# leggedrobotics/wild_visual_navigation

Hardware: NVIDIA H100
Metric: frames/sec end-to-end (DINO feat + seg + MLP train-step) at 448x448 (higher is better)
Workload: dtype bf16 operands / fp32 accumulate (ViT, STEGO head, per-pixel MLP); fp32 (k-means, train step)

## Files before the change

include/wvn_b200.h:

```cpp
#ifndef WVN_B200_H_
#define WVN_B200_H_

#include <stddef.h>
#include <stdint.h>

#ifdef __cplusplus
extern "C" {
#endif

typedef enum {
  WVN_STATUS_OK = 0,
  WVN_STATUS_INVALID = -1,
  WVN_STATUS_CUDA = -2,
  WVN_STATUS_NO_DEVICE = -3,
  WVN_STATUS_STATE = -4
} wvn_status;

const char* wvn_last_error(void);
int wvn_check_device(void);
int wvn_version(void);
long long wvn_launch_count(void);
void wvn_profile_enable(int category_mask);
int wvn_profile_collect(float* host_ms, long long* host_launches);

int wvn_gemm_bf16(const void* a_bf16, long long lda, const void* w_bf16, const float* bias, void* out, long long ldo,
                  int m, int n, int k, int out_kind, int act, int block_n, void* stream);

typedef struct {
  int m, n, k;
  int epi, act;
  int block_n;
  const void* a;
  long long lda;
  const void* w;
  const float* bias;
  void* out;
  long long ldo;
  const float* pos;
  int tokens_in, npad;
  int dim, heads;
  void* q_out;
  void* k_out;
  void* vt_out;
  int feat, trav_col;
  const void* x;
  long long ldx;
  float* trav;
  float* conf;
  float* loss_reco;
  const float* cg_mean;
  const float* cg_std;
  float cg_std_factor;
  int reverse_m;
  int registers;
  const void* residual;
  long long ldr;
} wvn_gemm_ex_args;
int wvn_gemm_bf16_ex(const wvn_gemm_ex_args* args, void* stream);

int wvn_attention_bf16(const void* q, const void* k, const void* vt, void* out, int batch, int heads, int npad,
                       int n_valid, float scale, void* stream);

int wvn_layernorm(const float* x, const float* gamma, const float* beta, void* out_bf16, long long rows, int dim,
                  float eps, void* stream);

typedef struct wvn_vit wvn_vit_t;

typedef struct {
  int image_size;
  int patch_size;
  int dim;
  int depth;
  int heads;
  int mlp_dim;
  int max_batch;
  int chunk;
  float ln_eps;
  int head_out;
  int registers;
} wvn_vit_config;

int wvn_vit_create(const wvn_vit_config* cfg, wvn_vit_t** out);
void wvn_vit_destroy(wvn_vit_t* h);

int wvn_vit_set_weight(wvn_vit_t* h, const char* name, const float* data, long long numel);

int wvn_vit_forward(wvn_vit_t* h, const float* img, int batch, int in_h, int in_w, int resized_h, int resized_w,
                    float* tokens_out, void* stream);

// ... 149 lines not shown
```

wild_visual_navigation_b200/_C.py:

```python
from __future__ import annotations

import ctypes
import os
from ctypes import POINTER, Structure, byref, c_char_p, c_float, c_int, c_longlong, c_size_t, c_void_p

import torch

_HERE = os.path.dirname(os.path.abspath(__file__))
LIB_PATH = os.environ.get("WVN_B200_LIB", os.path.join(_HERE, "libwvn_b200.so"))


class WvnError(RuntimeError):
    pass


class VitConfig(Structure):
    _fields_ = [
        ("image_size", c_int), ("patch_size", c_int), ("dim", c_int), ("depth", c_int), ("heads", c_int),
        ("mlp_dim", c_int), ("max_batch", c_int), ("chunk", c_int), ("ln_eps", c_float), ("head_out", c_int),
        ("registers", c_int),
    ]


class GemmExArgs(Structure):
    _fields_ = [
        ("m", c_int), ("n", c_int), ("k", c_int), ("epi", c_int), ("act", c_int), ("block_n", c_int),
        ("a", c_void_p), ("lda", c_longlong), ("w", c_void_p), ("bias", c_void_p), ("out", c_void_p), ("ldo", c_longlong),
        ("pos", c_void_p), ("tokens_in", c_int), ("npad", c_int), ("dim", c_int), ("heads", c_int),
        ("q_out", c_void_p), ("k_out", c_void_p), ("vt_out", c_void_p),
        ("feat", c_int), ("trav_col", c_int), ("x", c_void_p), ("ldx", c_longlong), ("trav", c_void_p),
        ("conf", c_void_p), ("loss_reco", c_void_p), ("cg_mean", c_void_p), ("cg_std", c_void_p),
        ("cg_std_factor", c_float), ("reverse_m", c_int), ("registers", c_int), ("residual", c_void_p), ("ldr", c_longlong),
    ]


class ResnetConfig(Structure):
    _fields_ = [("image_size", c_int), ("depth", c_int), ("max_batch", c_int)]


class TrainConfig(Structure):
    _fields_ = [
        ("w_trav", c_float), ("w_reco", c_float), ("std_factor", c_float), ("anomaly_balanced", c_int),
        ("lr", c_float), ("beta1", c_float), ("beta2", c_float), ("eps", c_float),
    ]


class FlowBuffers(Structure):
    _fields_ = [("mask0", c_void_p), ("mask1", c_void_p), ("p1", c_void_p), ("invp1", c_void_p), ("p3", c_void_p),
                ("invp3", c_void_p)]


_lib = None

_P, _I, _L, _F, _S = c_void_p, c_int, c_longlong, c_float, c_size_t
SIGNATURES = {
    "wvn_last_error": (c_char_p, []),
    "wvn_check_device": (_I, []),
    "wvn_version": (_I, []),
    "wvn_launch_count": (_L, []),
    "wvn_profile_enable": (None, [_I]),
    "wvn_profile_collect": (_I, [_P, _P]),
    "wvn_gemm_bf16": (_I, [_P, _L, _P, _P, _P, _L, _I, _I, _I, _I, _I, _I, _P]),
    "wvn_gemm_bf16_ex": (_I, [POINTER(GemmExArgs), _P]),
    "wvn_attention_bf16": (_I, [_P, _P, _P, _P, _I, _I, _I, _I, _F, _P]),
    "wvn_layernorm": (_I, [_P, _P, _P, _P, _L, _I, _F, _P]),
# ... 108 lines not shown
```

wild_visual_navigation_b200/csrc/api.cu:

```cuda
#include <cuda_bf16.h>

#include <stdio.h>
#include <stdlib.h>

#include <map>
#include <string>
#include <vector>

#include "../../include/wvn_b200.h"
#include "attention.h"
#include "dense_kernels.h"
#include "gemm.h"
#include "host_common.h"
#include "mlp_train.h"
#include "mlp_train_fused.h"
#include "pixel_head.h"
#include "resnet_kernels.h"
#include "segment_kernels.h"
#include "flow_train.h"
#include "footprint_kernels.h"
#include "slic_kernels.h"
#include "stego_kmeans.h"
#include "train_core.h"
#include "vit_kernels.h"
// ... 54 lines not shown
};

}

struct wvn_vit {
  wvn_vit_config cfg;
  int grid = 0, P = 0, t0 = 1, n_valid = 0, npad = 0, kpe = 0, kpe_ld = 0, chunk = 0;
  std::map<std::string, Weight> w;
  std::vector<DevBuf> owned;
  DevBuf x, xn, q, k, vt, attn, hid, ape, stage;
  DevBuf tok_bf16, head_hidden;
  DevBuf qkv_f32;
  bool precise = false;
  bool forwarded = false;
  int last_batch = 0;

  int add_weight(const std::string& name, long long numel, bool bf16, int cols = 0, int ld = 0) {
    DevBuf b;
    const long long stored = cols > 0 ? numel / cols * ld : numel;
    WVN_PROPAGATE(b.alloc(static_cast<size_t>(stored) * (bf16 ? 2 : 4)));
    owned.push_back(b);
    Weight wt;
    wt.p = b.p; wt.numel = numel; wt.bf16 = bf16; wt.cols = cols; wt.ld = ld;
    w[name] = wt;
    return WVN_OK;
  }
  template <class T>
  T* wp(const std::string& name) { return reinterpret_cast<T*>(w[name].p); }
};

extern "C" {

const char* wvn_last_error(void) { return last_error(); }
int wvn_version(void) { return 104; }

int wvn_check_device(void) {
  int n = 0;
  if (cudaGetDeviceCount(&n) != cudaSuccess || n == 0) return set_error(WVN_ERR_NO_DEVICE, "no CUDA device visible");
  int dev = 0;
  cudaGetDevice(&dev);
  int major = 0;
  cudaDeviceGetAttribute(&major, cudaDevAttrComputeCapabilityMajor, dev);
  int minor = 0;
  cudaDeviceGetAttribute(&minor, cudaDevAttrComputeCapabilityMinor, dev);
  if (major != 9 || minor != 0)
    return set_error(WVN_ERR_NO_DEVICE, "device %d has compute capability %d.%d, need 9.0 (sm_90a)", dev, major, minor);
  return WVN_OK;
}

long long wvn_launch_count(void) { return launch_count(); }
void wvn_profile_enable(int category_mask) { prof_enable(category_mask); }
int wvn_profile_collect(float* host_ms, long long* host_launches) {
  WVN_REQUIRE(host_ms && host_launches, "wvn_profile_collect: null argument");
  return prof_collect(host_ms, host_launches);
}

int wvn_gemm_bf16(const void* a, long long lda, const void* w, const float* bias, void* out, long long ldo, int m, int n,
                  int k, int out_kind, int act, int block_n, void* stream) {
  GemmArgs g;
  g.M = m; g.N = n; g.K = k;
  g.epi = out_kind == 0 ? EPI_BF16 : (out_kind == 1 ? EPI_F32 : EPI_RESID_F32);
  WVN_REQUIRE(out_kind >= 0 && out_kind <= 2, "wvn_gemm_bf16: out_kind %d", out_kind);
  g.act = act; g.bias = bias; g.out = out; g.ldo = ldo;
  return gemm_bf16(g, a, lda, w, block_n, S(stream));
}

int wvn_gemm_bf16_ex(const wvn_gemm_ex_args* x, void* stream) {
  WVN_REQUIRE(x, "wvn_gemm_bf16_ex: null argument");
  GemmArgs g;
  g.M = x->m; g.N = x->n; g.K = x->k; g.epi = x->epi; g.act = x->act;
  g.bias = x->bias; g.out = x->out; g.ldo = x->ldo;
  g.pos = x->pos; g.tokens_in = x->tokens_in; g.npad = x->npad;
  g.dim = x->dim; g.heads = x->heads; g.q = x->q_out; g.k = x->k_out; g.vt = x->vt_out;
  g.feat = x->feat; g.trav_col = x->trav_col; g.x = x->x; g.ldx = x->ldx; g.trav = x->trav; g.conf = x->conf;
  g.loss_reco = x->loss_reco; g.cg_mean = x->cg_mean; g.cg_std = x->cg_std; g.cg_std_factor = x->cg_std_factor;
  g.reverse_m = x->reverse_m; g.registers = x->registers;
  g.residual = x->residual; g.ldr = x->ldr;
  return gemm_bf16(g, x->a, x->lda, x->w, x->block_n, S(stream));
}

int wvn_attention_bf16(const void* q, const void* k, const void* vt, void* out, int batch, int heads, int npad,
                       int n_valid, float scale, void* stream) {
  AttnArgs a;
  a.batch = batch; a.heads = heads; a.npad = npad; a.n_valid = n_valid;
  a.scale_log2 = scale * 1.4426950408889634f;
  a.out = out; a.ldo = static_cast<long long>(heads) * 64;
  return attention_bf16(a, q, k, vt, S(stream));
}

int wvn_layernorm(const float* x, const float* gamma, const float* beta, void* out_bf16, long long rows, int dim,
                  float eps, void* stream) {
  LayerNormArgs a;
  a.rows = rows; a.dim = dim; a.eps = eps;
  return layernorm_rows(x, gamma, beta, out_bf16, nullptr, a, S(stream));
}

int wvn_vit_create(const wvn_vit_config* cfg, wvn_vit_t** out) {
  WVN_REQUIRE(cfg && out, "wvn_vit_create: null argument");
  WVN_PROPAGATE(wvn_check_device());
  WVN_REQUIRE(cfg->dim == 384 || cfg->dim == 768, "vit: dim %d unsupported (384, 768)", cfg->dim);
  WVN_REQUIRE(cfg->heads * 64 == cfg->dim, "vit: heads*64 must equal dim");
  WVN_REQUIRE(cfg->patch_size == 8 || cfg->patch_size == 14 || cfg->patch_size == 16, "vit: patch size %d unsupported",
              cfg->patch_size);
  WVN_REQUIRE(cfg->image_size >= cfg->patch_size, "vit: image size too small");
  WVN_REQUIRE(cfg->mlp_dim % 64 == 0 && cfg->depth > 0 && cfg->max_batch > 0, "vit: bad mlp_dim/depth/max_batch");
  WVN_REQUIRE(cfg->head_out % 64 == 0, "vit: head_out must be a multiple of 64");
  WVN_REQUIRE(cfg->registers >= 0, "vit: registers must be >= 0");
  WVN_REQUIRE(cfg->registers == 0 || cfg->head_out == 0, "vit: register tokens and a STEGO head cannot be combined");
  wvn_vit* h = new wvn_vit();
  h->cfg = *cfg;
  if (h->cfg.ln_eps <= 0.f) h->cfg.ln_eps = 1e-6f;
// ... 1146 lines not shown
```

wild_visual_navigation_b200/csrc/gemm.h:

```cpp
#pragma once

#include <cuda_runtime.h>

namespace wvn {

enum GemmEpilogue : int {
  EPI_BF16 = 0,
  EPI_F32 = 1,
  EPI_RESID_F32 = 2,
  EPI_PATCH = 3,
  EPI_QKV = 4,
  EPI_MLP_HEAD = 5,
  EPI_BF16_RESID = 6,
};

enum GemmAct : int { ACT_NONE = 0, ACT_RELU = 1, ACT_GELU = 2 };

struct GemmArgs {
  int M = 0, N = 0, K = 0;
  int epi = EPI_BF16, act = ACT_NONE;
  const float* bias = nullptr;
  void* out = nullptr;
  long long ldo = 0;
  const float* pos = nullptr;
  int tokens_in = 0;
  int registers = 0;
  int npad = 0;
  int dim = 0, heads = 0;
  void* q = nullptr;
  void* k = nullptr;
  void* vt = nullptr;
  int feat = 0;
  int trav_col = 0;
  const void* x = nullptr;
  long long ldx = 0;
  float* trav = nullptr;
  float* conf = nullptr;
  float* loss_reco = nullptr;
  const float* cg_mean = nullptr;
  const float* cg_std = nullptr;
  float cg_std_factor = 0.5f;
  const void* residual = nullptr;
  long long ldr = 0;
  int max_ctas = 0;
  int reverse_m = 0;
};

int pick_block_n(int N);

inline long long gemm_w_pitch(int K) { return (static_cast<long long>(K) + 7) / 8 * 8; }

int gemm_bf16(const GemmArgs& args, const void* A, long long lda, const void* W, int block_n, cudaStream_t stream);

}
```

wild_visual_navigation_b200/csrc/gemm_wgmma.cu:

```cuda
#include <stdlib.h>

#include <algorithm>

#include "common.cuh"
#include "gemm.h"
#include "host_common.h"

namespace wvn {

namespace {

constexpr int BM = 64;
constexpr int BK = 64;
constexpr int kConsumerWarps = 8;
constexpr int kNumThreads = 128 + kConsumerWarps * 32;
constexpr int kMaxSmemBytes = 227 * 1024;
constexpr int kMaxStages = 8;
constexpr int kFixedSmemBytes = 1024  + 1024 ;
constexpr int kSliceCols = 32;
constexpr int kResidMaxBlockN = 192;

template <bool ROW_OWNER>
struct TileIter {
  int num_m, num_n, m_blk, n_blk, lin;
  __device__ TileIter(int nm, int nn) : num_m(nm), num_n(nn), m_blk(0), n_blk(0), lin(0) {
    if (ROW_OWNER) { m_blk = blockIdx.x; n_blk = 0; }
    else { lin = blockIdx.x; m_blk = lin / num_n; n_blk = lin % num_n; }
  }
  __device__ bool valid() const { return m_blk < num_m; }
  __device__ void next() {
    if (ROW_OWNER) { if (++n_blk == num_n) { n_blk = 0; m_blk += gridDim.x; } }
    else { lin += gridDim.x; m_blk = lin / num_n; n_blk = lin % num_n; }
  }
};

template <int EPI>
constexpr bool kStaged = EPI == EPI_BF16 || EPI == EPI_F32 || EPI == EPI_RESID_F32 || EPI == EPI_QKV || EPI == EPI_BF16_RESID;

template <int BN, int EPI>
struct GemmCfg {
  static constexpr uint32_t kABytes = BM * BK * 2;
  static constexpr uint32_t kBBytes = BN * BK * 2;
  static constexpr uint32_t kStageBytes = kABytes + kBBytes;
  static constexpr uint32_t kSliceBytes = BM * kSliceCols * ((EPI == EPI_F32 || EPI == EPI_RESID_F32) ? 4 : 2);
  static constexpr uint32_t kStagingBytes = kStaged<EPI> ? 2 * 2 * kSliceBytes : 0;
  static constexpr int kStagesRaw = (kMaxSmemBytes - kFixedSmemBytes - kStagingBytes) / kStageBytes;
  static constexpr int kStages = kStagesRaw > kMaxStages ? kMaxStages : kStagesRaw;
  static constexpr uint32_t kSmemBytes = kStages * kStageBytes + kStagingBytes + kFixedSmemBytes;
  static constexpr int kN128 = BN / 128;
  static constexpr int kN64 = (BN % 128) / 64;
  static constexpr int kN32 = (BN % 64) / 32;
};

__device__ __forceinline__ float gelu_erf_fast(float x) {
  const float t = fminf(fabsf(x), 5.5f);
  float p = fmaf(-0.0003865310864f, t, 0.006509808358f);
  p = fmaf(p, t, -0.05048002675f);
  p = fmaf(p, t, -0.4613505006f);
  p = fmaf(p, t, -1.150225043f);
  p = fmaf(p, t, -1.00010848f);
  float e;
  asm("ex2.approx.ftz.f32 %0, %1;" : "=f"(e) : "f"(p));
  return fmaf(-t, e, fmaxf(x, 0.f));
}

template <int ACT>
__device__ __forceinline__ float activate(float v) {
  if (ACT == ACT_RELU) return fmaxf(v, 0.f);
  if (ACT == ACT_GELU) return gelu_erf_fast(v);
  return v;
}

template <int EPI, int ACT, int NREG>
__device__ __forceinline__ void epilogue_frag(const GemmArgs& args, const float (&d)[NREG], const int row0,
                                              const int col_base, const int lane, float (&head_partial)[2]) {
  const int q = lane & 3;
  bool ok[2];
  long long orow[2];
  int tok[2];
#pragma unroll
  for (int h = 0; h < 2; ++h) {
    const int row = row0 + 8 * h;
    ok[h] = row < args.M;
    orow[h] = row;
// ... 71 lines not shown
        }
        const float v0 = activate<ACT>(a0), v1 = activate<ACT>(a1);
        if (EPI == EPI_F32 || EPI == EPI_RESID_F32) {
          sts64(buf + r * 128 + ((((2 * js + (q >> 1)) ^ (r & 7))) << 4) + (q & 1) * 8, v0, v1);
        } else if (EPI == EPI_QKV && which == 2) {
          const int dd = 8 * js + 2 * q;
          const uint32_t t = 2 * r;
          sts16(buf + dd * 128 + (((t >> 4) ^ (dd & 7)) << 4) + (t & 15), __float2bfloat16_rn(v0));
          sts16(buf + (dd + 1) * 128 + (((t >> 4) ^ ((dd + 1) & 7)) << 4) + (t & 15), __float2bfloat16_rn(v1));
        } else {
          sts32(buf + r * 64 + ((js ^ ((r >> 1) & 3)) << 4) + q * 4, pack_bf16x2(v0, v1));
        }
      }
    }
    fence_proxy_async_smem();
    named_bar_sync(bar_id, 128);
    if (leader) {
      if (EPI == EPI_BF16 || EPI == EPI_F32 || EPI == EPI_BF16_RESID) {
        tma_store_2d(tm0, buf, col, row_tile);
      } else if (EPI == EPI_RESID_F32) {
        tma_reduce_add_2d(tm0, buf, col, row_tile);
      } else if (EPI == EPI_QKV) {
        const int frame = row_tile / args.npad;
        const int tok0 = row_tile - frame * args.npad;
        const int bh = frame * args.heads + (within >> 6);
        if (which < 2) tma_store_2d(which == 0 ? tm0 : tm1, buf, within & 63, bh * args.npad + tok0);
        else tma_store_2d(tm2, buf, tok0, bh * 64 + (within & 63));
      }
      tma_store_commit();
    }
  }
}

template <int BN, int EPI, int ACT>
__global__ void __launch_bounds__(kNumThreads, 1)
gemm_bf16_kernel(const __grid_constant__ CUtensorMap tmap_a, const __grid_constant__ CUtensorMap tmap_b,
                 const __grid_constant__ CUtensorMap tmap_c0, const __grid_constant__ CUtensorMap tmap_c1,
                 const __grid_constant__ CUtensorMap tmap_c2, const GemmArgs args) {
  using Cfg = GemmCfg<BN, EPI>;
  constexpr int STAGES = Cfg::kStages;

  extern __shared__ uint8_t smem_raw[];
  uint8_t* smem = reinterpret_cast<uint8_t*>((reinterpret_cast<uintptr_t>(smem_raw) + 1023) & ~uintptr_t(1023));
  uint8_t* smem_b = smem;
  uint8_t* smem_a = smem + STAGES * Cfg::kBBytes;
  uint8_t* smem_c = smem_a + STAGES * Cfg::kABytes;
  uint64_t* bars = reinterpret_cast<uint64_t*>(smem_c + Cfg::kStagingBytes);
  uint64_t* full_bar = bars;
  uint64_t* empty_bar = bars + kMaxStages;

  const int warp = threadIdx.x >> 5;
  const int lane = threadIdx.x & 31;

  const int num_m = (args.M + BM - 1) / BM;
  const int num_n = args.N / BN;
  const int num_k = (args.K + BK - 1) / BK;
  constexpr bool ROW_OWNER = (EPI == EPI_MLP_HEAD);

  if (threadIdx.x == 0) {
    tma_prefetch_desc(&tmap_a);
    tma_prefetch_desc(&tmap_b);
    for (int i = 0; i < kMaxStages; ++i) {
      mbar_init(&full_bar[i], 1);
      mbar_init(&empty_bar[i], kConsumerWarps / 2);
    }
    fence_mbar_init();
  }
  __syncthreads();

  if (warp < 4) {
    setmaxnreg_dec<40>();
    if (warp == 0) {
      int stage = 0;
      uint32_t phase = 0;
      for (TileIter<ROW_OWNER> it(num_m, num_n); it.valid(); it.next()) {
        const int m_eff = args.reverse_m ? num_m - 1 - it.m_blk : it.m_blk;
        for (int kb = 0; kb < num_k; ++kb) {
          mbar_wait(&empty_bar[stage], phase ^ 1);
          if (elect_one_sync()) {
            mbar_arrive_expect_tx(&full_bar[stage], Cfg::kStageBytes);
            tma_load_2d(&tmap_a, &full_bar[stage], smem_a + stage * Cfg::kABytes, kb * BK, m_eff * BM);
            tma_load_2d(&tmap_b, &full_bar[stage], smem_b + stage * Cfg::kBBytes, kb * BK, it.n_blk * BN);
          }
          __syncwarp();
          if (++stage == STAGES) { stage = 0; phase ^= 1; }
        }
      }
    }
  } else {
    setmaxnreg_inc<232>();
    const int cwarp = warp - 4;
    const int wg = cwarp >> 2;
    const int row_local = (cwarp & 3) * 16 + (lane >> 2);
    const bool leader = (threadIdx.x & 127) == 0;
    const uint32_t staging = smem_u32(smem_c) + wg * 2 * Cfg::kSliceBytes;
    if (kStaged<EPI> && leader) {
      tma_prefetch_desc(&tmap_c0);
      if (EPI == EPI_QKV) {
        tma_prefetch_desc(&tmap_c1);
        tma_prefetch_desc(&tmap_c2);
      }
    }
    if (wg == 1) named_bar_arrive(1, 256);
    float acc128[Cfg::kN128 > 0 ? Cfg::kN128 : 1][64];
    float acc64[32];
    float acc32[16];
    float head_partial[2] = {0.f, 0.f};
    int stage = 0;
    uint32_t phase = 0;
    int unit = 0;
    for (TileIter<ROW_OWNER> it(num_m, num_n); it.valid(); it.next()) {
      const bool unit_end = !ROW_OWNER || it.n_blk == num_n - 1;
      if ((unit & 1) != wg) {
        for (int kb = 0; kb < num_k; ++kb)
          if (++stage == STAGES) { stage = 0; phase ^= 1; }
        if (unit_end) ++unit;
        continue;
      }
      if (!ROW_OWNER || it.n_blk == 0) named_bar_sync(1 + wg, 256);
      int prev_stage = 0;
      for (int kb = 0; kb < num_k; ++kb) {
        mbar_wait(&full_bar[stage], phase);
        const uint64_t desc_a = make_sw128_kmajor_desc(smem_u32(smem_a + stage * Cfg::kABytes));
        const uint32_t b_addr = smem_u32(smem_b + stage * Cfg::kBBytes);
#pragma unroll
        for (int c = 0; c < Cfg::kN128; ++c) wgmma_fence_regs(acc128[c]);
        if (Cfg::kN64) wgmma_fence_regs(acc64);
        if (Cfg::kN32) wgmma_fence_regs(acc32);
        wgmma_fence();
#pragma unroll
        for (int k = 0; k < BK / 16; ++k) {
          const uint32_t accumulate = (kb | k) != 0 ? 1u : 0u;
#pragma unroll
          for (int c = 0; c < Cfg::kN128; ++c)
            wgmma_m64n128k16_ss(acc128[c], desc_a + 2 * k, make_sw128_kmajor_desc(b_addr + c * 128 * 128) + 2 * k, accumulate);
          if (Cfg::kN64)
            wgmma_m64n64k16_ss(acc64, desc_a + 2 * k, make_sw128_kmajor_desc(b_addr + Cfg::kN128 * 128 * 128) + 2 * k, accumulate);
          if (Cfg::kN32)
            wgmma_m64n32k16_ss(acc32, desc_a + 2 * k,
                               make_sw128_kmajor_desc(b_addr + (Cfg::kN128 * 128 + Cfg::kN64 * 64) * 128) + 2 * k, accumulate);
        }
        wgmma_commit();
        if (kb > 0) {
          wgmma_wait<1>();
          if (lane == 0) mbar_arrive(&empty_bar[prev_stage]);
        }
        prev_stage = stage;
        if (++stage == STAGES) { stage = 0; phase ^= 1; }
      }
      if (unit_end && (ROW_OWNER ? it.m_blk + static_cast<int>(gridDim.x) < num_m : it.lin + static_cast<int>(gridDim.x) < num_m * num_n))
        named_bar_arrive(2 - wg, 256);
      wgmma_wait<0>();
#pragma unroll
      for (int c = 0; c < Cfg::kN128; ++c) wgmma_fence_regs(acc128[c]);
      if (Cfg::kN64) wgmma_fence_regs(acc64);
      if (Cfg::kN32) wgmma_fence_regs(acc32);
      if (lane == 0) mbar_arrive(&empty_bar[prev_stage]);

      const int m_eff = args.reverse_m ? num_m - 1 - it.m_blk : it.m_blk;
      const int row_tile = m_eff * BM;
      const int col0 = it.n_blk * BN;
      if (kStaged<EPI>) {
        const int bar_id = 3 + wg;
#pragma unroll
        for (int c = 0; c < Cfg::kN128; ++c)
          store_frag<EPI, ACT>(args, &tmap_c0, &tmap_c1, &tmap_c2, acc128[c], row_tile, col0 + c * 128, row_local, lane,
                               leader, bar_id, staging, Cfg::kSliceBytes, 4 * c);
        if (Cfg::kN64)
          store_frag<EPI, ACT>(args, &tmap_c0, &tmap_c1, &tmap_c2, acc64, row_tile, col0 + Cfg::kN128 * 128, row_local,
                               lane, leader, bar_id, staging, Cfg::kSliceBytes, 4 * Cfg::kN128);
        if (Cfg::kN32)
          store_frag<EPI, ACT>(args, &tmap_c0, &tmap_c1, &tmap_c2, acc32, row_tile, col0 + Cfg::kN128 * 128 + Cfg::kN64 * 64,
                               row_local, lane, leader, bar_id, staging, Cfg::kSliceBytes, 4 * Cfg::kN128 + 2 * Cfg::kN64);
      } else {
        const int row0 = row_tile + row_local;
#pragma unroll
        for (int c = 0; c < Cfg::kN128; ++c)
          epilogue_frag<EPI, ACT>(args, acc128[c], row0, col0 + c * 128, lane, head_partial);
        if (Cfg::kN64) epilogue_frag<EPI, ACT>(args, acc64, row0, col0 + Cfg::kN128 * 128, lane, head_partial);
        if (Cfg::kN32) epilogue_frag<EPI, ACT>(args, acc32, row0, col0 + Cfg::kN128 * 128 + Cfg::kN64 * 64, lane, head_partial);
      }

      if (EPI == EPI_MLP_HEAD && it.n_blk == num_n - 1) {
#pragma unroll
        for (int h = 0; h < 2; ++h) {
          float s = head_partial[h];
          s += __shfl_xor_sync(0xffffffffu, s, 1);
          s += __shfl_xor_sync(0xffffffffu, s, 2);
          head_partial[h] = 0.f;
          const int row = row_tile + row_local + 8 * h;
          if ((lane & 3) == 0 && row < args.M) {
            const float loss = s / static_cast<float>(args.feat);
            const float mean = __ldg(args.cg_mean), sd = __ldg(args.cg_std);
            const float shifted = mean + sd * args.cg_std_factor;
            const float lo = fmaxf(shifted - sd, 0.f);
            const float hi = shifted + sd;
            const float xc = fminf(fmaxf(loss, lo), hi);
            args.conf[row] = 1.f - (xc - lo) / (hi - lo);
            if (args.loss_reco != nullptr) args.loss_reco[row] = loss;
          }
        }
      }
      if (unit_end) ++unit;
    }
    if (kStaged<EPI> && leader) tma_store_wait_all<0>();
  }
}

template <int BN, int EPI, int ACT>
int launch_gemm(const GemmArgs& a, const CUtensorMap& ta, const CUtensorMap& tb, const CUtensorMap (&tc)[3],
                cudaStream_t stream) {
  using Cfg = GemmCfg<BN, EPI>;
  static_assert(Cfg::kStages >= 2, "tile too wide for the shared-memory budget");
  auto kern = gemm_bf16_kernel<BN, EPI, ACT>;
  static bool attr_set = false;
  if (!attr_set) {
    WVN_CHECK_CUDA(cudaFuncSetAttribute(kern, cudaFuncAttributeMaxDynamicSharedMemorySize, kMaxSmemBytes));
    attr_set = true;
  }
  const int num_m = (a.M + BM - 1) / BM, num_n = a.N / BN;
  const int num_tiles = (EPI == EPI_MLP_HEAD) ? num_m : num_m * num_n;
  int grid = sm_count();
  if (a.max_ctas > 0 && a.max_ctas < grid) grid = a.max_ctas;
  if (grid > num_tiles) grid = num_tiles;
  prof_begin(PROF_GEMM, stream);
  kern<<<grid, kNumThreads, Cfg::kSmemBytes, stream>>>(ta, tb, tc[0], tc[1], tc[2], a);
  prof_end(PROF_GEMM, stream);
  WVN_CHECK_LAUNCH("gemm_bf16_kernel");
  return WVN_OK;
}

template <int BN>
int dispatch_epi(const GemmArgs& a, const CUtensorMap& ta, const CUtensorMap& tb, const CUtensorMap (&tc)[3],
                 cudaStream_t s) {
  switch (a.epi) {
    case EPI_BF16:
      if (a.act == ACT_NONE) return launch_gemm<BN, EPI_BF16, ACT_NONE>(a, ta, tb, tc, s);
      if (a.act == ACT_RELU) return launch_gemm<BN, EPI_BF16, ACT_RELU>(a, ta, tb, tc, s);
      if (a.act == ACT_GELU) return launch_gemm<BN, EPI_BF16, ACT_GELU>(a, ta, tb, tc, s);
      break;
    case EPI_F32:
      if (a.act == ACT_NONE) return launch_gemm<BN, EPI_F32, ACT_NONE>(a, ta, tb, tc, s);
      break;
    case EPI_RESID_F32:
      if (a.act == ACT_NONE) return launch_gemm<BN, EPI_RESID_F32, ACT_NONE>(a, ta, tb, tc, s);
      break;
    case EPI_PATCH:
      if (a.act == ACT_NONE) return launch_gemm<BN, EPI_PATCH, ACT_NONE>(a, ta, tb, tc, s);
      break;
    case EPI_QKV:
      if (a.act == ACT_NONE) return launch_gemm<BN, EPI_QKV, ACT_NONE>(a, ta, tb, tc, s);
      break;
    case EPI_MLP_HEAD:
      if (a.act == ACT_NONE) return launch_gemm<BN, EPI_MLP_HEAD, ACT_NONE>(a, ta, tb, tc, s);
      break;
    case EPI_BF16_RESID:
      if constexpr (BN <= kResidMaxBlockN) {
        if (a.act == ACT_NONE) return launch_gemm<BN, EPI_BF16_RESID, ACT_NONE>(a, ta, tb, tc, s);
        if (a.act == ACT_RELU) return launch_gemm<BN, EPI_BF16_RESID, ACT_RELU>(a, ta, tb, tc, s);
      }
      break;
  }
  return set_error(WVN_ERR_INVALID, "gemm: unsupported epilogue/activation combination (%d, %d)", a.epi, a.act);
}

}

int pick_block_n(int N) {
  if (N % 256 == 0) return 256;
  if (N % 224 == 0) return 224;
  if (N % 192 == 0) return 192;
  if (N % 128 == 0) return 128;
  if (N % 64 == 0) return 64;
  return 0;
}

int gemm_bf16(const GemmArgs& a, const void* A, long long lda, const void* W, int block_n, cudaStream_t stream) {
  WVN_REQUIRE(a.M > 0 && a.N > 0 && a.K > 0, "gemm: empty problem (M=%d N=%d K=%d)", a.M, a.N, a.K);
  WVN_REQUIRE(lda >= a.K, "gemm: lda=%lld is smaller than K=%d", lda, a.K);
  if (block_n == 0) {
    block_n = pick_block_n(a.N);
    if (a.epi == EPI_BF16_RESID && block_n > kResidMaxBlockN) block_n = a.N % 192 == 0 ? 192 : (a.N % 128 == 0 ? 128 : 64);
  }
  WVN_REQUIRE(a.epi != EPI_BF16_RESID || block_n <= kResidMaxBlockN, "gemm: the residual epilogue takes block_n <= %d",
              kResidMaxBlockN);
  WVN_REQUIRE(block_n == 64 || block_n == 128 || block_n == 192 || block_n == 224 || block_n == 256,
              "gemm: bad block_n %d", block_n);
  WVN_REQUIRE(a.N % block_n == 0, "gemm: N=%d must be a multiple of block_n=%d (pad the weights)", a.N, block_n);
  if (a.epi == EPI_MLP_HEAD)
    WVN_REQUIRE(a.feat > 0 && a.trav_col % 32 == 0 && a.trav_col >= a.feat && a.trav_col < a.N && a.x != nullptr &&
                    a.trav != nullptr && a.conf != nullptr && a.cg_mean != nullptr && a.cg_std != nullptr &&
                    a.ldx % 8 == 0 && a.ldx >= a.trav_col,
                "gemm: bad MLP-head epilogue arguments (feat=%d trav_col=%d N=%d)", a.feat, a.trav_col, a.N);
  if (a.epi == EPI_QKV)
    WVN_REQUIRE(a.dim % 64 == 0 && a.N == 3 * a.dim && a.heads * 64 == a.dim && a.npad % 8 == 0 && a.npad % BM == 0 &&
                    a.M % a.npad == 0,
                "gemm: bad QKV epilogue geometry (dim=%d heads=%d npad=%d N=%d M=%d)", a.dim, a.heads, a.npad, a.N, a.M);
  if (a.epi == EPI_PATCH)
    WVN_REQUIRE(a.tokens_in > 0 && a.registers >= 0 && 1 + a.registers + a.tokens_in <= a.npad,
                "gemm: bad patch-embed epilogue geometry (tokens_in=%d registers=%d npad=%d)", a.tokens_in, a.registers,
                a.npad);
  if (a.epi == EPI_F32 || a.epi == EPI_RESID_F32) WVN_REQUIRE(a.ldo % 4 == 0, "gemm: fp32 output pitch must be a multiple of 4");
  if (a.epi == EPI_BF16 || a.epi == EPI_BF16_RESID) WVN_REQUIRE(a.ldo % 8 == 0, "gemm: bf16 output pitch must be a multiple of 8");
  if (a.epi == EPI_BF16_RESID)
    WVN_REQUIRE(a.residual != nullptr && a.ldr >= a.N && a.ldr % 2 == 0,
                "gemm: the residual epilogue needs a bf16 residual with an even pitch ldr >= N (ldr=%lld N=%d)", a.ldr, a.N);
  CUtensorMap ta, tb, tc[3] = {};
  WVN_PROPAGATE(make_tmap_bf16_2d(&ta, A, a.K, a.M, static_cast<uint64_t>(lda) * 2, BK, BM));
  WVN_PROPAGATE(make_tmap_bf16_2d(&tb, W, a.K, a.N, static_cast<uint64_t>(gemm_w_pitch(a.K)) * 2, BK, block_n));
  if (a.epi == EPI_BF16 || a.epi == EPI_BF16_RESID)
    WVN_PROPAGATE(make_tmap_2d(&tc[0], a.out, 2, a.N, a.M, static_cast<uint64_t>(a.ldo) * 2, kSliceCols, BM, 64));
  if (a.epi == EPI_F32 || a.epi == EPI_RESID_F32)
    WVN_PROPAGATE(make_tmap_2d(&tc[0], a.out, 4, a.N, a.M, static_cast<uint64_t>(a.ldo) * 4, kSliceCols, BM, 128));
  if (a.epi == EPI_QKV) {
    const uint64_t bh = static_cast<uint64_t>(a.M / a.npad) * a.heads;
    WVN_PROPAGATE(make_tmap_2d(&tc[0], a.q, 2, 64, bh * a.npad, 128, kSliceCols, BM, 64));
    WVN_PROPAGATE(make_tmap_2d(&tc[1], a.k, 2, 64, bh * a.npad, 128, kSliceCols, BM, 64));
    WVN_PROPAGATE(make_tmap_2d(&tc[2], a.vt, 2, a.npad, bh * 64, static_cast<uint64_t>(a.npad) * 2, BM, kSliceCols, 128));
  }
  switch (block_n) {
    case 64: return dispatch_epi<64>(a, ta, tb, tc, stream);
    case 128: return dispatch_epi<128>(a, ta, tb, tc, stream);
    case 192: return dispatch_epi<192>(a, ta, tb, tc, stream);
    case 224: return dispatch_epi<224>(a, ta, tb, tc, stream);
    case 256: return dispatch_epi<256>(a, ta, tb, tc, stream);
  }
  return set_error(WVN_ERR_INVALID, "gemm: unreachable");
}

}
```

Measured before the change: 972.5.

## Add 128-row GEMM tiles with a wave-cost tile picker for staged epilogues

Templates the wgmma GEMM kernel on block_m so each consumer warpgroup can hold two 64-row accumulator halves, giving 128-row tiles. Each B tile loaded from shared memory is then reused across twice as many rows. A picker compares wave-quantised tile costs and falls back to 64 rows for small-K problems and for epilogues that cannot take tall tiles. The risks are higher register pressure from the doubled accumulators, fewer pipeline stages, and less parallelism on small GEMMs. It also removes the max_ctas grid cap and changes the default block_n choice for some shapes.

Result: faster. 985.6 (median of 6 runs) (+1.3%).

```diff
diff --git a/include/wvn_b200.h b/include/wvn_b200.h
--- a/include/wvn_b200.h
+++ b/include/wvn_b200.h
@@ -55,6 +55,7 @@
   int registers;
   const void* residual;
   long long ldr;
+  int block_m;
 } wvn_gemm_ex_args;
 int wvn_gemm_bf16_ex(const wvn_gemm_ex_args* args, void* stream);
 
diff --git a/wild_visual_navigation_b200/_C.py b/wild_visual_navigation_b200/_C.py
--- a/wild_visual_navigation_b200/_C.py
+++ b/wild_visual_navigation_b200/_C.py
@@ -31,6 +31,7 @@
         ("feat", c_int), ("trav_col", c_int), ("x", c_void_p), ("ldx", c_longlong), ("trav", c_void_p),
         ("conf", c_void_p), ("loss_reco", c_void_p), ("cg_mean", c_void_p), ("cg_std", c_void_p),
         ("cg_std_factor", c_float), ("reverse_m", c_int), ("registers", c_int), ("residual", c_void_p), ("ldr", c_longlong),
+        ("block_m", c_int),
     ]
 
 
diff --git a/wild_visual_navigation_b200/csrc/api.cu b/wild_visual_navigation_b200/csrc/api.cu
--- a/wild_visual_navigation_b200/csrc/api.cu
+++ b/wild_visual_navigation_b200/csrc/api.cu
@@ -110,7 +110,7 @@
 extern "C" {
 
 const char* wvn_last_error(void) { return last_error(); }
-int wvn_version(void) { return 104; }
+int wvn_version(void) { return 105; }
 
 int wvn_check_device(void) {
   int n = 0;
@@ -154,7 +154,7 @@
   g.loss_reco = x->loss_reco; g.cg_mean = x->cg_mean; g.cg_std = x->cg_std; g.cg_std_factor = x->cg_std_factor;
   g.reverse_m = x->reverse_m; g.registers = x->registers;
   g.residual = x->residual; g.ldr = x->ldr;
-  return gemm_bf16(g, x->a, x->lda, x->w, x->block_n, S(stream));
+  return gemm_bf16(g, x->a, x->lda, x->w, x->block_n, S(stream), x->block_m);
 }
 
 int wvn_attention_bf16(const void* q, const void* k, const void* vt, void* out, int batch, int heads, int npad,
diff --git a/wild_visual_navigation_b200/csrc/gemm.h b/wild_visual_navigation_b200/csrc/gemm.h
--- a/wild_visual_navigation_b200/csrc/gemm.h
+++ b/wild_visual_navigation_b200/csrc/gemm.h
@@ -42,14 +42,17 @@
   float cg_std_factor = 0.5f;
   const void* residual = nullptr;
   long long ldr = 0;
-  int max_ctas = 0;
   int reverse_m = 0;
 };
 
 int pick_block_n(int N);
 
+bool tall_tiles_ok(const GemmArgs& args);
+void pick_tile(const GemmArgs& args, int sms, int& block_m, int& block_n);
+
 inline long long gemm_w_pitch(int K) { return (static_cast<long long>(K) + 7) / 8 * 8; }
 
-int gemm_bf16(const GemmArgs& args, const void* A, long long lda, const void* W, int block_n, cudaStream_t stream);
+int gemm_bf16(const GemmArgs& args, const void* A, long long lda, const void* W, int block_n, cudaStream_t stream,
+              int block_m = 0);
 
 }
diff --git a/wild_visual_navigation_b200/csrc/gemm_wgmma.cu b/wild_visual_navigation_b200/csrc/gemm_wgmma.cu
--- a/wild_visual_navigation_b200/csrc/gemm_wgmma.cu
+++ b/wild_visual_navigation_b200/csrc/gemm_wgmma.cu
@@ -10,7 +10,7 @@
 
 namespace {
 
-constexpr int BM = 64;
+constexpr int kHalfRows = 64;
 constexpr int BK = 64;
 constexpr int kConsumerWarps = 8;
 constexpr int kNumThreads = 128 + kConsumerWarps * 32;
@@ -19,6 +19,8 @@
 constexpr int kFixedSmemBytes = 1024  + 1024 ;
 constexpr int kSliceCols = 32;
 constexpr int kResidMaxBlockN = 192;
+constexpr int kTallMaxBlockN = 128;
+constexpr int kTallMinKPerOutByte = 384;
 
 template <bool ROW_OWNER>
 struct TileIter {
@@ -37,12 +39,16 @@
 template <int EPI>
 constexpr bool kStaged = EPI == EPI_BF16 || EPI == EPI_F32 || EPI == EPI_RESID_F32 || EPI == EPI_QKV || EPI == EPI_BF16_RESID;
 
-template <int BN, int EPI>
+template <int EPI>
+constexpr bool kTallOk = EPI == EPI_BF16 || EPI == EPI_F32 || EPI == EPI_RESID_F32 || EPI == EPI_QKV;
+
+template <int BN, int EPI, int BM>
 struct GemmCfg {
+  static constexpr int kHalves = BM / kHalfRows;
   static constexpr uint32_t kABytes = BM * BK * 2;
   static constexpr uint32_t kBBytes = BN * BK * 2;
   static constexpr uint32_t kStageBytes = kABytes + kBBytes;
-  static constexpr uint32_t kSliceBytes = BM * kSliceCols * ((EPI == EPI_F32 || EPI == EPI_RESID_F32) ? 4 : 2);
+  static constexpr uint32_t kSliceBytes = kHalfRows * kSliceCols * ((EPI == EPI_F32 || EPI == EPI_RESID_F32) ? 4 : 2);
   static constexpr uint32_t kStagingBytes = kStaged<EPI> ? 2 * 2 * kSliceBytes : 0;
   static constexpr int kStagesRaw = (kMaxSmemBytes - kFixedSmemBytes - kStagingBytes) / kStageBytes;
   static constexpr int kStages = kStagesRaw > kMaxStages ? kMaxStages : kStagesRaw;
@@ -50,6 +56,7 @@
   static constexpr int kN128 = BN / 128;
   static constexpr int kN64 = (BN % 128) / 64;
   static constexpr int kN32 = (BN % 64) / 32;
+  static constexpr int kSlicesPerHalf = BN / kSliceCols;
 };
 
 __device__ __forceinline__ float gelu_erf_fast(float x) {
@@ -187,13 +194,15 @@
   }
 }
 
-template <int BN, int EPI, int ACT>
+template <int BN, int EPI, int ACT, int BM>
 __global__ void __launch_bounds__(kNumThreads, 1)
 gemm_bf16_kernel(const __grid_constant__ CUtensorMap tmap_a, const __grid_constant__ CUtensorMap tmap_b,
                  const __grid_constant__ CUtensorMap tmap_c0, const __grid_constant__ CUtensorMap tmap_c1,
                  const __grid_constant__ CUtensorMap tmap_c2, const GemmArgs args) {
-  using Cfg = GemmCfg<BN, EPI>;
+  static_assert(BM == kHalfRows || (BM == 2 * kHalfRows && kTallOk<EPI>), "128-row tiles take the staged epilogues only");
+  using Cfg = GemmCfg<BN, EPI, BM>;
   constexpr int STAGES = Cfg::kStages;
+  constexpr int HM = Cfg::kHalves;
 
   extern __shared__ uint8_t smem_raw[];
   uint8_t* smem = reinterpret_cast<uint8_t*>((reinterpret_cast<uintptr_t>(smem_raw) + 1023) & ~uintptr_t(1023));
@@ -257,9 +266,9 @@
       }
     }
     if (wg == 1) named_bar_arrive(1, 256);
-    float acc128[Cfg::kN128 > 0 ? Cfg::kN128 : 1][64];
-    float acc64[32];
-    float acc32[16];
+    float acc128[HM][Cfg::kN128 > 0 ? Cfg::kN128 : 1][64];
+    float acc64[HM][32];
+    float acc32[HM][16];
     float head_partial[2] = {0.f, 0.f};
     int stage = 0;
     uint32_t phase = 0;
@@ -276,24 +285,33 @@
       int prev_stage = 0;
       for (int kb = 0; kb < num_k; ++kb) {
         mbar_wait(&full_bar[stage], phase);
-        const uint64_t desc_a = make_sw128_kmajor_desc(smem_u32(smem_a + stage * Cfg::kABytes));
+        const uint32_t a_addr = smem_u32(smem_a + stage * Cfg::kABytes);
         const uint32_t b_addr = smem_u32(smem_b + stage * Cfg::kBBytes);
 #pragma unroll
-        for (int c = 0; c < Cfg::kN128; ++c) wgmma_fence_regs(acc128[c]);
-        if (Cfg::kN64) wgmma_fence_regs(acc64);
-        if (Cfg::kN32) wgmma_fence_regs(acc32);
+        for (int h = 0; h < HM; ++h) {
+#pragma unroll
+          for (int c = 0; c < Cfg::kN128; ++c) wgmma_fence_regs(acc128[h][c]);
+          if (Cfg::kN64) wgmma_fence_regs(acc64[h]);
+          if (Cfg::kN32) wgmma_fence_regs(acc32[h]);
+        }
         wgmma_fence();
 #pragma unroll
         for (int k = 0; k < BK / 16; ++k) {
           const uint32_t accumulate = (kb | k) != 0 ? 1u : 0u;
 #pragma unroll
-          for (int c = 0; c < Cfg::kN128; ++c)
-            wgmma_m64n128k16_ss(acc128[c], desc_a + 2 * k, make_sw128_kmajor_desc(b_addr + c * 128 * 128) + 2 * k, accumulate);
-          if (Cfg::kN64)
-            wgmma_m64n64k16_ss(acc64, desc_a + 2 * k, make_sw128_kmajor_desc(b_addr + Cfg::kN128 * 128 * 128) + 2 * k, accumulate);
-          if (Cfg::kN32)
-            wgmma_m64n32k16_ss(acc32, desc_a + 2 * k,
-                               make_sw128_kmajor_desc(b_addr + (Cfg::kN128 * 128 + Cfg::kN64 * 64) * 128) + 2 * k, accumulate);
+          for (int h = 0; h < HM; ++h) {
+            const uint64_t desc_a = make_sw128_kmajor_desc(a_addr + h * kHalfRows * BK * 2) + 2 * k;
+#pragma unroll
+            for (int c = 0; c < Cfg::kN128; ++c)
+              wgmma_m64n128k16_ss(acc128[h][c], desc_a, make_sw128_kmajor_desc(b_addr + c * 128 * 128) + 2 * k, accumulate);
+            if (Cfg::kN64)
+              wgmma_m64n64k16_ss(acc64[h], desc_a, make_sw128_kmajor_desc(b_addr + Cfg::kN128 * 128 * 128) + 2 * k,
+                                 accumulate);
+            if (Cfg::kN32)
+              wgmma_m64n32k16_ss(acc32[h], desc_a,
+                                 make_sw128_kmajor_desc(b_addr + (Cfg::kN128 * 128 + Cfg::kN64 * 64) * 128) + 2 * k,
+                                 accumulate);
+          }
         }
         wgmma_commit();
         if (kb > 0) {
@@ -307,9 +325,12 @@
         named_bar_arrive(2 - wg, 256);
       wgmma_wait<0>();
 #pragma unroll
-      for (int c = 0; c < Cfg::kN128; ++c) wgmma_fence_regs(acc128[c]);
-      if (Cfg::kN64) wgmma_fence_regs(acc64);
-      if (Cfg::kN32) wgmma_fence_regs(acc32);
+      for (int h = 0; h < HM; ++h) {
+#pragma unroll
+        for (int c = 0; c < Cfg::kN128; ++c) wgmma_fence_regs(acc128[h][c]);
+        if (Cfg::kN64) wgmma_fence_regs(acc64[h]);
+        if (Cfg::kN32) wgmma_fence_regs(acc32[h]);
+      }
       if (lane == 0) mbar_arrive(&empty_bar[prev_stage]);
 
       const int m_eff = args.reverse_m ? num_m - 1 - it.m_blk : it.m_blk;
@@ -318,22 +339,29 @@
       if (kStaged<EPI>) {
         const int bar_id = 3 + wg;
 #pragma unroll
-        for (int c = 0; c < Cfg::kN128; ++c)
-          store_frag<EPI, ACT>(args, &tmap_c0, &tmap_c1, &tmap_c2, acc128[c], row_tile, col0 + c * 128, row_local, lane,
-                               leader, bar_id, staging, Cfg::kSliceBytes, 4 * c);
-        if (Cfg::kN64)
-          store_frag<EPI, ACT>(args, &tmap_c0, &tmap_c1, &tmap_c2, acc64, row_tile, col0 + Cfg::kN128 * 128, row_local,
-                               lane, leader, bar_id, staging, Cfg::kSliceBytes, 4 * Cfg::kN128);
-        if (Cfg::kN32)
-          store_frag<EPI, ACT>(args, &tmap_c0, &tmap_c1, &tmap_c2, acc32, row_tile, col0 + Cfg::kN128 * 128 + Cfg::kN64 * 64,
-                               row_local, lane, leader, bar_id, staging, Cfg::kSliceBytes, 4 * Cfg::kN128 + 2 * Cfg::kN64);
+        for (int h = 0; h < HM; ++h) {
+          const int row_h = row_tile + h * kHalfRows;
+          const int slice0 = h * Cfg::kSlicesPerHalf;
+#pragma unroll
+          for (int c = 0; c < Cfg::kN128; ++c)
+            store_frag<EPI, ACT>(args, &tmap_c0, &tmap_c1, &tmap_c2, acc128[h][c], row_h, col0 + c * 128, row_local,
+                                 lane, leader, bar_id, staging, Cfg::kSliceBytes, slice0 + 4 * c);
+          if (Cfg::kN64)
+            store_frag<EPI, ACT>(args, &tmap_c0, &tmap_c1, &tmap_c2, acc64[h], row_h, col0 + Cfg::kN128 * 128, row_local,
+                                 lane, leader, bar_id, staging, Cfg::kSliceBytes, slice0 + 4 * Cfg::kN128);
+          if (Cfg::kN32)
+            store_frag<EPI, ACT>(args, &tmap_c0, &tmap_c1, &tmap_c2, acc32[h], row_h,
+                                 col0 + Cfg::kN128 * 128 + Cfg::kN64 * 64, row_local, lane, leader, bar_id, staging,
+                                 Cfg::kSliceBytes, slice0 + 4 * Cfg::kN128 + 2 * Cfg::kN64);
+        }
       } else {
         const int row0 = row_tile + row_local;
 #pragma unroll
         for (int c = 0; c < Cfg::kN128; ++c)
-          epilogue_frag<EPI, ACT>(args, acc128[c], row0, col0 + c * 128, lane, head_partial);
-        if (Cfg::kN64) epilogue_frag<EPI, ACT>(args, acc64, row0, col0 + Cfg::kN128 * 128, lane, head_partial);
-        if (Cfg::kN32) epilogue_frag<EPI, ACT>(args, acc32, row0, col0 + Cfg::kN128 * 128 + Cfg::kN64 * 64, lane, head_partial);
+          epilogue_frag<EPI, ACT>(args, acc128[0][c], row0, col0 + c * 128, lane, head_partial);
+        if (Cfg::kN64) epilogue_frag<EPI, ACT>(args, acc64[0], row0, col0 + Cfg::kN128 * 128, lane, head_partial);
+        if (Cfg::kN32)
+          epilogue_frag<EPI, ACT>(args, acc32[0], row0, col0 + Cfg::kN128 * 128 + Cfg::kN64 * 64, lane, head_partial);
       }
 
       if (EPI == EPI_MLP_HEAD && it.n_blk == num_n - 1) {
@@ -362,12 +390,12 @@
   }
 }
 
-template <int BN, int EPI, int ACT>
+template <int BN, int EPI, int ACT, int BM>
 int launch_gemm(const GemmArgs& a, const CUtensorMap& ta, const CUtensorMap& tb, const CUtensorMap (&tc)[3],
                 cudaStream_t stream) {
-  using Cfg = GemmCfg<BN, EPI>;
+  using Cfg = GemmCfg<BN, EPI, BM>;
   static_assert(Cfg::kStages >= 2, "tile too wide for the shared-memory budget");
-  auto kern = gemm_bf16_kernel<BN, EPI, ACT>;
+  auto kern = gemm_bf16_kernel<BN, EPI, ACT, BM>;
   static bool attr_set = false;
   if (!attr_set) {
     WVN_CHECK_CUDA(cudaFuncSetAttribute(kern, cudaFuncAttributeMaxDynamicSharedMemorySize, kMaxSmemBytes));
@@ -375,9 +403,7 @@
   }
   const int num_m = (a.M + BM - 1) / BM, num_n = a.N / BN;
   const int num_tiles = (EPI == EPI_MLP_HEAD) ? num_m : num_m * num_n;
-  int grid = sm_count();
-  if (a.max_ctas > 0 && a.max_ctas < grid) grid = a.max_ctas;
-  if (grid > num_tiles) grid = num_tiles;
+  const int grid = std::min(sm_count(), num_tiles);
   prof_begin(PROF_GEMM, stream);
   kern<<<grid, kNumThreads, Cfg::kSmemBytes, stream>>>(ta, tb, tc[0], tc[1], tc[2], a);
   prof_end(PROF_GEMM, stream);
@@ -385,36 +411,40 @@
   return WVN_OK;
 }
 
-template <int BN>
+template <int BN, int BM>
 int dispatch_epi(const GemmArgs& a, const CUtensorMap& ta, const CUtensorMap& tb, const CUtensorMap (&tc)[3],
                  cudaStream_t s) {
   switch (a.epi) {
     case EPI_BF16:
-      if (a.act == ACT_NONE) return launch_gemm<BN, EPI_BF16, ACT_NONE>(a, ta, tb, tc, s);
-      if (a.act == ACT_RELU) return launch_gemm<BN, EPI_BF16, ACT_RELU>(a, ta, tb, tc, s);
-      if (a.act == ACT_GELU) return launch_gemm<BN, EPI_BF16, ACT_GELU>(a, ta, tb, tc, s);
+      if (a.act == ACT_NONE) return launch_gemm<BN, EPI_BF16, ACT_NONE, BM>(a, ta, tb, tc, s);
+      if (a.act == ACT_RELU) return launch_gemm<BN, EPI_BF16, ACT_RELU, BM>(a, ta, tb, tc, s);
+      if (a.act == ACT_GELU) return launch_gemm<BN, EPI_BF16, ACT_GELU, BM>(a, ta, tb, tc, s);
       break;
     case EPI_F32:
-      if (a.act == ACT_NONE) return launch_gemm<BN, EPI_F32, ACT_NONE>(a, ta, tb, tc, s);
+      if (a.act == ACT_NONE) return launch_gemm<BN, EPI_F32, ACT_NONE, BM>(a, ta, tb, tc, s);
       break;
     case EPI_RESID_F32:
-      if (a.act == ACT_NONE) return launch_gemm<BN, EPI_RESID_F32, ACT_NONE>(a, ta, tb, tc, s);
-      break;
-    case EPI_PATCH:
-      if (a.act == ACT_NONE) return launch_gemm<BN, EPI_PATCH, ACT_NONE>(a, ta, tb, tc, s);
+      if (a.act == ACT_NONE) return launch_gemm<BN, EPI_RESID_F32, ACT_NONE, BM>(a, ta, tb, tc, s);
       break;
     case EPI_QKV:
-      if (a.act == ACT_NONE) return launch_gemm<BN, EPI_QKV, ACT_NONE>(a, ta, tb, tc, s);
+      if (a.act == ACT_NONE) return launch_gemm<BN, EPI_QKV, ACT_NONE, BM>(a, ta, tb, tc, s);
       break;
-    case EPI_MLP_HEAD:
-      if (a.act == ACT_NONE) return launch_gemm<BN, EPI_MLP_HEAD, ACT_NONE>(a, ta, tb, tc, s);
-      break;
-    case EPI_BF16_RESID:
-      if constexpr (BN <= kResidMaxBlockN) {
-        if (a.act == ACT_NONE) return launch_gemm<BN, EPI_BF16_RESID, ACT_NONE>(a, ta, tb, tc, s);
-        if (a.act == ACT_RELU) return launch_gemm<BN, EPI_BF16_RESID, ACT_RELU>(a, ta, tb, tc, s);
-      }
-      break;
+  }
+  if constexpr (BM == kHalfRows) {
+    switch (a.epi) {
+      case EPI_PATCH:
+        if (a.act == ACT_NONE) return launch_gemm<BN, EPI_PATCH, ACT_NONE, BM>(a, ta, tb, tc, s);
+        break;
+      case EPI_MLP_HEAD:
+        if (a.act == ACT_NONE) return launch_gemm<BN, EPI_MLP_HEAD, ACT_NONE, BM>(a, ta, tb, tc, s);
+        break;
+      case EPI_BF16_RESID:
+        if constexpr (BN <= kResidMaxBlockN) {
+          if (a.act == ACT_NONE) return launch_gemm<BN, EPI_BF16_RESID, ACT_NONE, BM>(a, ta, tb, tc, s);
+          if (a.act == ACT_RELU) return launch_gemm<BN, EPI_BF16_RESID, ACT_RELU, BM>(a, ta, tb, tc, s);
+        }
+        break;
+    }
   }
   return set_error(WVN_ERR_INVALID, "gemm: unsupported epilogue/activation combination (%d, %d)", a.epi, a.act);
 }
@@ -430,13 +460,64 @@
   return 0;
 }
 
-int gemm_bf16(const GemmArgs& a, const void* A, long long lda, const void* W, int block_n, cudaStream_t stream) {
+bool tall_tiles_ok(const GemmArgs& a) {
+  return (a.epi == EPI_BF16 || a.epi == EPI_F32 || a.epi == EPI_RESID_F32 || a.epi == EPI_QKV) &&
+         (a.epi != EPI_QKV || a.npad % 128 == 0);
+}
+
+static long long tile_cost(int M, int N, int block_m, int block_n, int sms) {
+  const long long tiles = static_cast<long long>((M + block_m - 1) / block_m) * (N / block_n);
+  return (tiles + sms - 1) / sms * (block_m + block_n);
+}
+
+void pick_tile(const GemmArgs& a, int sms, int& block_m, int& block_n) {
+  const int out_bytes = (a.epi == EPI_F32 || a.epi == EPI_RESID_F32) ? 4 : 2;
+  if (block_m == 64 || !tall_tiles_ok(a)) {
+    block_m = 64;
+    if (block_n == 0) block_n = pick_block_n(a.N);
+    return;
+  }
+  if (block_m == 0 && a.K < kTallMinKPerOutByte * out_bytes) {
+    block_m = 64;
+    if (block_n == 0) block_n = a.K < 768 && a.N % 192 == 0 ? 192 : pick_block_n(a.N);
+    return;
+  }
+  int best_m = 0, best_n = 0;
+  long long best = 0;
+  auto consider = [&](int bm, int bn) {
+    if (bn == 0 || a.N % bn != 0) return;
+    const long long c = tile_cost(a.M, a.N, bm, bn, sms);
+    if (best_m == 0 || c < best) {
+      best = c;
+      best_m = bm;
+      best_n = bn;
+    }
+  };
+  if (block_m == 0) consider(64, block_n != 0 ? block_n : pick_block_n(a.N));
+  if (block_n != 0) {
+    if (block_n <= kTallMaxBlockN) consider(128, block_n);
+  } else {
+    for (const int bn : {128, 64}) consider(128, bn);
+  }
+  block_m = best_m;
+  block_n = best_n;
+}
+
+int gemm_bf16(const GemmArgs& a, const void* A, long long lda, const void* W, int block_n, cudaStream_t stream,
+              int block_m) {
   WVN_REQUIRE(a.M > 0 && a.N > 0 && a.K > 0, "gemm: empty problem (M=%d N=%d K=%d)", a.M, a.N, a.K);
   WVN_REQUIRE(lda >= a.K, "gemm: lda=%lld is smaller than K=%d", lda, a.K);
-  if (block_n == 0) {
+  WVN_REQUIRE(block_m == 0 || block_m == 64 || block_m == 128, "gemm: bad block_m %d", block_m);
+  WVN_REQUIRE(block_m != 128 || tall_tiles_ok(a),
+              "gemm: block_m 128 takes the bf16, fp32, residual-add and QKV epilogues (QKV with npad %% 128 == 0); "
+              "epi=%d npad=%d", a.epi, a.npad);
+  WVN_REQUIRE(block_m != 128 || block_n <= kTallMaxBlockN, "gemm: block_m 128 takes block_n <= %d (block_n=%d)",
+              kTallMaxBlockN, block_n);
+  if (block_n == 0 && a.epi == EPI_BF16_RESID) {
     block_n = pick_block_n(a.N);
-    if (a.epi == EPI_BF16_RESID && block_n > kResidMaxBlockN) block_n = a.N % 192 == 0 ? 192 : (a.N % 128 == 0 ? 128 : 64);
-  }
+    if (block_n > kResidMaxBlockN) block_n = a.N % 192 == 0 ? 192 : (a.N % 128 == 0 ? 128 : 64);
+  }
+  pick_tile(a, sm_count(), block_m, block_n);
   WVN_REQUIRE(a.epi != EPI_BF16_RESID || block_n <= kResidMaxBlockN, "gemm: the residual epilogue takes block_n <= %d",
               kResidMaxBlockN);
   WVN_REQUIRE(block_n == 64 || block_n == 128 || block_n == 192 || block_n == 224 || block_n == 256,
@@ -448,7 +529,8 @@
                     a.ldx % 8 == 0 && a.ldx >= a.trav_col,
                 "gemm: bad MLP-head epilogue arguments (feat=%d trav_col=%d N=%d)", a.feat, a.trav_col, a.N);
   if (a.epi == EPI_QKV)
-    WVN_REQUIRE(a.dim % 64 == 0 && a.N == 3 * a.dim && a.heads * 64 == a.dim && a.npad % 8 == 0 && a.npad % BM == 0 &&
+    WVN_REQUIRE(a.dim % 64 == 0 && a.N == 3 * a.dim && a.heads * 64 == a.dim && a.npad % 8 == 0 &&
+                    a.npad % block_m == 0 &&
                     a.M % a.npad == 0,
                 "gemm: bad QKV epilogue geometry (dim=%d heads=%d npad=%d N=%d M=%d)", a.dim, a.heads, a.npad, a.N, a.M);
   if (a.epi == EPI_PATCH)
@@ -461,24 +543,30 @@
     WVN_REQUIRE(a.residual != nullptr && a.ldr >= a.N && a.ldr % 2 == 0,
                 "gemm: the residual epilogue needs a bf16 residual with an even pitch ldr >= N (ldr=%lld N=%d)", a.ldr, a.N);
   CUtensorMap ta, tb, tc[3] = {};
-  WVN_PROPAGATE(make_tmap_bf16_2d(&ta, A, a.K, a.M, static_cast<uint64_t>(lda) * 2, BK, BM));
+  WVN_PROPAGATE(make_tmap_bf16_2d(&ta, A, a.K, a.M, static_cast<uint64_t>(lda) * 2, BK, block_m));
   WVN_PROPAGATE(make_tmap_bf16_2d(&tb, W, a.K, a.N, static_cast<uint64_t>(gemm_w_pitch(a.K)) * 2, BK, block_n));
   if (a.epi == EPI_BF16 || a.epi == EPI_BF16_RESID)
-    WVN_PROPAGATE(make_tmap_2d(&tc[0], a.out, 2, a.N, a.M, static_cast<uint64_t>(a.ldo) * 2, kSliceCols, BM, 64));
+    WVN_PROPAGATE(make_tmap_2d(&tc[0], a.out, 2, a.N, a.M, static_cast<uint64_t>(a.ldo) * 2, kSliceCols, kHalfRows, 64));
   if (a.epi == EPI_F32 || a.epi == EPI_RESID_F32)
-    WVN_PROPAGATE(make_tmap_2d(&tc[0], a.out, 4, a.N, a.M, static_cast<uint64_t>(a.ldo) * 4, kSliceCols, BM, 128));
+    WVN_PROPAGATE(make_tmap_2d(&tc[0], a.out, 4, a.N, a.M, static_cast<uint64_t>(a.ldo) * 4, kSliceCols, kHalfRows, 128));
   if (a.epi == EPI_QKV) {
     const uint64_t bh = static_cast<uint64_t>(a.M / a.npad) * a.heads;
-    WVN_PROPAGATE(make_tmap_2d(&tc[0], a.q, 2, 64, bh * a.npad, 128, kSliceCols, BM, 64));
-    WVN_PROPAGATE(make_tmap_2d(&tc[1], a.k, 2, 64, bh * a.npad, 128, kSliceCols, BM, 64));
-    WVN_PROPAGATE(make_tmap_2d(&tc[2], a.vt, 2, a.npad, bh * 64, static_cast<uint64_t>(a.npad) * 2, BM, kSliceCols, 128));
+    WVN_PROPAGATE(make_tmap_2d(&tc[0], a.q, 2, 64, bh * a.npad, 128, kSliceCols, kHalfRows, 64));
+    WVN_PROPAGATE(make_tmap_2d(&tc[1], a.k, 2, 64, bh * a.npad, 128, kSliceCols, kHalfRows, 64));
+    WVN_PROPAGATE(make_tmap_2d(&tc[2], a.vt, 2, a.npad, bh * 64, static_cast<uint64_t>(a.npad) * 2, kHalfRows, kSliceCols, 128));
+  }
+  if (block_m == 128) {
+    switch (block_n) {
+      case 64: return dispatch_epi<64, 128>(a, ta, tb, tc, stream);
+      case 128: return dispatch_epi<128, 128>(a, ta, tb, tc, stream);
+    }
   }
   switch (block_n) {
-    case 64: return dispatch_epi<64>(a, ta, tb, tc, stream);
-    case 128: return dispatch_epi<128>(a, ta, tb, tc, stream);
-    case 192: return dispatch_epi<192>(a, ta, tb, tc, stream);
-    case 224: return dispatch_epi<224>(a, ta, tb, tc, stream);
-    case 256: return dispatch_epi<256>(a, ta, tb, tc, stream);
+    case 64: return dispatch_epi<64, 64>(a, ta, tb, tc, stream);
+    case 128: return dispatch_epi<128, 64>(a, ta, tb, tc, stream);
+    case 192: return dispatch_epi<192, 64>(a, ta, tb, tc, stream);
+    case 224: return dispatch_epi<224, 64>(a, ta, tb, tc, stream);
+    case 256: return dispatch_epi<256, 64>(a, ta, tb, tc, stream);
   }
   return set_error(WVN_ERR_INVALID, "gemm: unreachable");
 }
```
